# hermda02/dang

Measured on AMD Instinct MI355X. Metric: gibbs_iterations_per_sec, higher is better.
Workload: dtype f64

## Files before the change

### dang_amd/csrc/dangx_planeset.hip

```cpp
#ifndef DX_NO_VCOEF
#define DX_VCOEF 1
#endif
#include "dx_host.h"
#include "dx_kern_planeset.h"

static size_t planeset_lds(int ng, int nb, int nv, int lanes, int Sp) {
    const int rows = nv > Sp ? nv : Sp;
    return ((size_t)(TROWS * ng + 3) * nb + (size_t)rows * (nb / lanes) * BLOCK) * sizeof(double);
}

static void item_codes(const SweepList& sl, int code[4]) {
    for (int q = 0; q < 4; ++q) code[q] = (q < sl.n) ? sl.s[q].mode + 8 * sl.s[q].pair : 0;
}
static std::string planeset_name(int Sp, int nb, int ng, int lanes, int solve, const SweepList& sl, int bp) {
    int c[4];
    item_codes(sl, c);
    std::string s = "dxk::k_plane_set<" + std::to_string(Sp) + ", " + std::to_string(nb) + ", " + std::to_string(ng) + ", " + std::to_string(lanes) +
                    ", " + std::to_string(solve);
    for (int q = 0; q < 4; ++q) s += ", " + std::to_string(c[q]);
    return s + ", " + std::to_string(bp) + ">";
}

static int planeset_bp(dangx_ctx* ctx) {
    for (int j = 0; j < ctx->hm.nbands; ++j)
        if (ctx->hm.band[j].n != 0) return 1;
    return 0;
}

static bool planeset_builtin(int nb, int ng, int lanes, int solve, const SweepList& sl) {
    int c[4];
    item_codes(sl, c);
    if (nb == 20 && ng == 6 && lanes == 2) return solve && c[0] == CH_POW && c[1] == CH_MBB_BETA + 8 && c[2] == CH_LOGN_NUP && c[3] == 0;
    if (lanes == 1 && nb == 10 && ng == 4 && solve && sl.n == 0) return true;
    if (lanes == 1 && ((nb == 10 && ng == 4) || (solve && ((nb == 5 && ng == 3) || (nb == 3 && ng == 2)))))
        return c[0] == CH_POW && c[1] == CH_MBB_BETA + 8 && c[2] == 0 && c[3] == 0;
    return false;
}

template <int NB, int NG, int LP, int SOLVE, int C0, int C1, int C2>
static void launch_builtin(dangx_ctx* ctx, const GroupArgs& ga, const FusedArgs& fa, const SweepList& sl, int Sp, unsigned nblk, size_t ldsz,
                           unsigned long long* accp) {
    if (Sp == 2)
        hipLaunchKernelGGL((dxk::k_plane_set<2, NB, NG, LP, SOLVE, C0, C1, C2, 0>), dim3(nblk), dim3(BLOCK), ldsz, ctx->stream, ctx->dm, ga, fa, sl, ctx->counters, accp, ctx->partial);
    else
        hipLaunchKernelGGL((dxk::k_plane_set<1, NB, NG, LP, SOLVE, C0, C1, C2, 0>), dim3(nblk), dim3(BLOCK), ldsz, ctx->stream, ctx->dm, ga, fa, sl, ctx->counters, accp, ctx->partial);
}

static bool planeset_args(dangx_ctx* ctx, const GroupArgs& ga, const SweepList& sl, FusedArgs& fa) {
    fa.nv = 0; fa.gself = -1;
    unsigned planes = 0;
    for (int k = sl.s1; k <= sl.s2; ++k) planes |= 1u << (k - 1);
    for (int g = 0; g < MAXG; ++g) { fa.vslot[g] = -1; fa.vcomp[g] = 0; fa.vtype[g] = 0; }
    for (int g = 0; g < ga.ng; ++g) {
        const int l = ga.gc[g];
        const Comp& c = ctx->hm.comp[l];
        const unsigned cm = (unsigned)c.const_planes & planes;
        if (cm != 0 && cm != planes) return false;
        if (cm != planes) {
            if (c.type != DANGX_POWERLAW && c.type != DANGX_MBB && c.type != DANGX_FREEFREE && c.type != DANGX_LOGNORMAL) return false;
            if (sl.s2 > sl.s1 && (ctx->qu_equal[l] & ((1u << c.nind) - 1u)) != ((1u << c.nind) - 1u)) return false;
            fa.vcomp[fa.nv] = (signed char)g; fa.vtype[fa.nv] = (signed char)c.type;
            fa.vslot[g] = (signed char)fa.nv++;
        }
    }
    fa.cal = 0;
    if (sl.s1 == 1)
        for (int j = 0; j < ctx->hm.nbands; ++j)
            if (ctx->hm.gain[j] != 1.0 || ctx->hm.offset[j] != 0.0) fa.cal = 1;
    return true;
}

int dx_planeset_lanes(dangx_ctx* ctx, const GroupArgs& ga, const SweepList& sl, int solve) {
    static const bool enabled = [] { const char* e = getenv("DANGX_PLANESET"); return !(e && e[0] == '0'); }();
    static const bool small_too = [] { const char* e = getenv("DANGX_PLANESET"); return !(e && e[0] == 'p'); }();
    if (!enabled || sl.n < 0 || sl.n > 4 || (sl.n == 0 && !solve) || ga.ng < 1 || ga.ng > 6) return 0;
    static const int cap2 = [] { const char* e = getenv("DANGX_PS_CAP2"); return e ? atoi(e) : 13; }();
    const int nb = ctx->hm.nbands, Sp = sl.s2 - sl.s1 + 1, cap = (Sp == 2) ? cap2 : 16;
    for (int q = 0; q < sl.n; ++q) {
        const int m = sl.s[q].mode;
        if (m < CH_POW || m > CH_LOGN_W) return 0;
        if (sl.s[q].pair && !(m == CH_MBB_BETA || m == CH_LOGN_NUP)) return 0;
    }
    FusedArgs fa;
    if (!planeset_args(ctx, ga, sl, fa)) return 0;
    if (solve && fa.cal && ga.nuc > 0) return 0;
    const int bp = planeset_bp(ctx);
    if (bp) {
        for (int q = 0; q < sl.n; ++q)
            if (sl.s[q].mode > CH_MBB_T) return 0;
        if (!(small_too && nb <= cap && planeset_lds(ga.ng, nb, fa.nv, 1, Sp) <= 80u * 1024u)) return 0;
        return dx_rtc_get(ctx, "dx_kern_planeset.h", planeset_name(Sp, nb, ga.ng, 1, solve, sl, 1)) ? 1 : 0;
    }
    int lanes = 0;
    if (small_too && nb <= cap && planeset_lds(ga.ng, nb, fa.nv, 1, Sp) <= 80u * 1024u) lanes = 1;
    else if (nb > 12 && nb % 2 == 0 && nb / 2 <= cap && planeset_lds(ga.ng, nb, fa.nv, 2, Sp) <= 80u * 1024u) lanes = 2;
    if (!lanes) return 0;
    if (planeset_builtin(nb, ga.ng, lanes, solve, sl)) return lanes;
    return dx_rtc_get(ctx, "dx_kern_planeset.h", planeset_name(Sp, nb, ga.ng, lanes, solve, sl, 0)) ? lanes : 0;
}

bool dx_launch_planeset(dangx_ctx* ctx, const GroupArgs& ga, const SweepList& sl, int lanes, int solve, unsigned nblk, unsigned long long* accp) {
    FusedArgs fa;
    if (lanes < 1 || lanes > 2 || !planeset_args(ctx, ga, sl, fa)) return false;
    const int nb = ctx->hm.nbands, ng = ga.ng, Sp = sl.s2 - sl.s1 + 1;
    const size_t ldsz = planeset_lds(ng, nb, fa.nv, lanes, Sp);
    const int bp = planeset_bp(ctx);
    if (!bp && planeset_builtin(nb, ng, lanes, solve, sl)) {
        if (nb == 20) launch_builtin<20, 6, 2, 1, CH_POW, CH_MBB_BETA + 8, CH_LOGN_NUP>(ctx, ga, fa, sl, Sp, nblk, ldsz, accp);
        else if (nb == 10 && sl.n == 0) launch_builtin<10, 4, 1, 1, 0, 0, 0>(ctx, ga, fa, sl, Sp, nblk, ldsz, accp);
        else if (nb == 10 && !solve) launch_builtin<10, 4, 1, 0, CH_POW, CH_MBB_BETA + 8, 0>(ctx, ga, fa, sl, Sp, nblk, ldsz, accp);
        else if (nb == 10) launch_builtin<10, 4, 1, 1, CH_POW, CH_MBB_BETA + 8, 0>(ctx, ga, fa, sl, Sp, nblk, ldsz, accp);
        else if (nb == 5) launch_builtin<5, 3, 1, 1, CH_POW, CH_MBB_BETA + 8, 0>(ctx, ga, fa, sl, Sp, nblk, ldsz, accp);
        else launch_builtin<3, 2, 1, 1, CH_POW, CH_MBB_BETA + 8, 0>(ctx, ga, fa, sl, Sp, nblk, ldsz, accp);
        return true;
    }
    hipFunction_t fn = dx_rtc_get(ctx, "dx_kern_planeset.h", planeset_name(Sp, nb, ng, lanes, solve, sl, bp));
    if (!fn) return false;
    const Model* dm = ctx->dm;
    GroupArgs gg = ga;
    SweepList ss = sl;
    unsigned long long* bad = ctx->counters;
    double* part = ctx->partial;
    void* args[] = {&dm, &gg, &fa, &ss, &bad, &accp, &part};
    return dx_rtc_launch(ctx, fn, nblk, ldsz, args) == 0;
}
```

### dang_amd/csrc/dx_chain.h

```cpp
#pragma once
#include "dx_args.h"


template <bool V> struct BoolTag { static constexpr bool value = V; };

#ifdef DX_CHAIN_LIBEXP
#define CEXP(x) exp(x)
#define CEXPS(x) exp(x)
#define CEXP1(x) exp(x)
#else
#define CEXP(x) exp_nr(x)
#define CEXPS(x) exp_sat(x)
#define CEXP1(x) exp_nr_v(x)
#endif
#ifdef DX_CHAIN_IEEEDIV
#define CDIV(a, b) ((a) / (b))
#else
#define CDIV(a, b) ((a) * fast_rcp(b))
#endif

#ifndef DX_CHAIN_UNSCALED
#define DX_CHAIN_SCALED 1
#endif
#ifndef DX_CHAIN_PAIR_RNG
#define DX_CHAIN_PAIR_RNG 1
#endif

namespace {

__device__ __forceinline__ bool mh_accept(double diff, double u3) {
#if defined(DX_ACCEPT_FULL) || defined(DX_CHAIN_LIBEXP)
    return (diff >= 0.0) || (CEXP1(diff) > u3);
#else
    const float e = __builtin_amdgcn_exp2f((float)diff * 0x1.715476p+0f);
    const float uf = (float)u3;
    bool acc = (diff >= 0.0) || (e > uf * 0x1.001p+0f);
    const bool unsure = !(acc || e < uf * 0x1.ffep-1f);
    if (__builtin_amdgcn_ballot_w64(unsure) != 0ull) {
        if (unsure) acc = CEXP1(diff) > u3;
    }
    return acc;
#endif
}


template <int LP>
struct BandPick {
    int half;
    __device__ __forceinline__ double operator()(const double* arr, int j, int nbh) const {
        if (LP == 1) return arr[j];
        const double a = arr[j], b = arr[nbh + j];
        return half ? b : a;
    }
    __device__ __forceinline__ double nu_c(const Model& M, int j, int nbh) const {
        if (LP == 1) return M.band[j].nu_c;
        const double a = M.band[j].nu_c, b = M.band[nbh + j].nu_c;
        return half ? b : a;
    }
};

template <int MODE, int SP, int NB, int LP, bool KT = false, bool BP = false>
struct RegChain {
    static constexpr bool kBP = BP;
    double D[SP][NB], F[NB], ISr[SP][NB];
    double bpa, bpb;
    double K1[(LP > 1 && !KT) ? NB : 1], K2[(LP > 1 && !KT) ? NB : 1];
    const double *kt1, *kt2;
    double amp[SP];

    __device__ __forceinline__ double is(int kk, int j) const { return ISr[kk][j]; }
    __device__ __forceinline__ void set_is(int kk, int j, double v) { ISr[kk][j] = v; }
    __device__ __forceinline__ double k1(const Model& M, const Comp& c, int j) const {
        if (KT) return kt1[j];
        if (LP > 1) return K1[j];
        return (MODE == CH_MBB_T) ? M.band[j].nu_c : (MODE == CH_LOGN_NUP) ? c.lnu9[j] : c.lnr[j];
    }
    __device__ __forceinline__ double k2(const Comp& c, int j) const { return KT ? kt2[j] : (LP > 1) ? K2[j] : c.cst[j]; }
    __device__ __forceinline__ void set_kt(const double* tab, int nbands, int ng, int g, int jb) {
        kt1 = tab + ((MODE == CH_MBB_T) ? TROWS * ng : (MODE == CH_LOGN_NUP) ? TROWS * g + 2 : TROWS * g) * nbands + jb;
        kt2 = tab + (TROWS * g + 1) * nbands + jb;
    }
    __device__ __forceinline__ void set_k(const Model& M, const Comp& c, const BandPick<LP>& pick) {
        if (LP > 1 && !KT) {
#pragma unroll
            for (int j = 0; j < NB; ++j) {
                K1[j] = (MODE == CH_MBB_T) ? pick.nu_c(M, j, NB) : (MODE == CH_LOGN_NUP) ? pick(c.lnu9, j, NB) : pick(c.lnr, j, NB);
                K2[j] = (MODE == CH_LOGN_NUP || MODE == CH_LOGN_W) ? pick(c.cst, j, NB) : 0.0;
            }
        }
    }

    template <bool BATCH, int OP = 0>
    __device__ __forceinline__ double lnl(const Model& M, const Comp& c, double th, double other, double& acc0, double& acc1) {
        double s0 = 0.0, s1 = 0.0;
        if (MODE == CH_POW) s0 = th;
        else if (MODE == CH_MBB_BETA) s0 = th + 1.0;
        else if (MODE == CH_MBB_T) { s0 = mbb_z(th); s1 = CEXP(s0 * c.nu_ref) - 1.0; }
        else if (MODE == CH_LOGN_NUP) { s0 = log_pos(th); s1 = other; }
        else s1 = th;
        acc0 = 0.0; acc1 = 0.0;
#ifdef DX_CHAIN_IEEEDIV
        const double rs1 = 1.0 / s1;
#else
        const double rs1 = (MODE == CH_LOGN_NUP || MODE == CH_LOGN_W) ? fast_rcp(s1) : 0.0;
#endif
        constexpr int TT = BP ? 1 : (NB % 5 == 0) ? 5 : (NB % 4 == 0) ? 4 : (NB % 3 == 0) ? 3 : 1;
        static_assert(!BP || (LP == 1 && (MODE == CH_POW || MODE == CH_MBB_BETA || MODE == CH_MBB_T)), "bandpass chains: one lane, power law / mbb");
#pragma unroll
        for (int j0 = 0; j0 < NB; j0 += TT) {
            double s[TT];
            if (BP && M.band[j0].n != 0) {
                const Band& b = M.band[j0];
                const kptr nu = as_const(M.bp_nu0 + b.off);
                const kptr tau = as_const(M.bp_tau0 + b.off);
                const kptr lnr = as_const(c.bp_lnr + b.off);
                const int n = b.n;
                double sj = 0.0;
                if (MODE == CH_POW) {
#pragma unroll 4
                    for (int q = 0; q < n; ++q) sj = sj + tau[q] * CEXP(s0 * lnr[q]);
                } else if (MODE == CH_MBB_BETA) {
#pragma unroll 4
                    for (int q = 0; q < n; ++q) sj = sj + (tau[q] * bpb) * fast_rcp(CEXP(bpa * nu[q]) - 1.0) * CEXP(s0 * lnr[q]);
                } else {
#pragma unroll 4
                    for (int q = 0; q < n; ++q) sj = sj + (tau[q] * s1) * fast_rcp(CEXP(s0 * nu[q]) - 1.0) * CEXP(bpa * lnr[q]);
                }
                s[0] = sj;
            } else
            if (MODE == CH_MBB_T && TT > 1 && BATCH) {
                double den[TT], pre[TT];
#pragma unroll
                for (int t = 0; t < TT; ++t) den[t] = CEXP(s0 * k1(M, c, j0 + t)) - 1.0;
                pre[0] = den[0];
#pragma unroll
                for (int t = 1; t < TT; ++t) pre[t] = pre[t - 1] * den[t];
                double inv = s1 * fast_rcp(pre[TT - 1]);
#pragma unroll
                for (int t = TT - 1; t > 0; --t) {
                    s[t] = (inv * pre[t - 1]) * F[j0 + t];
                    inv *= den[t];
                }
                s[0] = inv * F[j0];
            } else
#pragma unroll
            for (int t = 0; t < TT; ++t) {
                const int j = j0 + t;
                if (MODE == CH_LOGN_NUP) {
                    const double l = (k1(M, c, j) - s0) * rs1;
                    s[t] = CEXPS(-0.5 * (l * l)) * k2(c, j);
                } else if (MODE == CH_LOGN_W) {
                    const double l = F[j] * rs1;
                    s[t] = CEXPS(-0.5 * (l * l)) * k2(c, j);
                } else {
                    const double e = CEXP(s0 * k1(M, c, j));
                    if (MODE == CH_POW) s[t] = e;
                    else if (MODE == CH_MBB_BETA) s[t] = F[j] * e;
                    else s[t] = CDIV(s1, e - 1.0) * F[j];
                }
            }
#pragma unroll
            for (int t = 0; t < TT; ++t) {
                const int j = j0 + t;
#ifdef DX_CHAIN_SCALED
                if (OP == 1) {
                    const double r0 = D[0][j];
                    D[0][j] = fma(is(0, j), s[t], r0);
                    acc0 = fma(r0, r0, acc0);
                    if (SP == 2) {
                        const double r1 = D[SP - 1][j];
                        D[SP - 1][j] = fma(is(SP - 1, j), s[t], r1);
                        acc1 = fma(r1, r1, acc1);
                    }
                } else if (OP == 2) {
                    D[0][j] = fma(-is(0, j), s[t], D[0][j]);
                    if (SP == 2) D[SP - 1][j] = fma(-is(SP - 1, j), s[t], D[SP - 1][j]);
                } else {
                const double r0 = fma(-is(0, j), s[t], D[0][j]);
                acc0 = fma(r0, r0, acc0);
                if (SP == 2) {
                    const double r1 = fma(-is(SP - 1, j), s[t], D[SP - 1][j]);
                    acc1 = fma(r1, r1, acc1);
                }
                }
#else
                const double r0 = (D[0][j] - amp[0] * s[t]) * is(0, j);
                acc0 = acc0 - 0.5 * (r0 * r0);
                if (SP == 2) {
                    const double r1 = (D[SP - 1][j] - amp[SP - 1] * s[t]) * is(SP - 1, j);
                    acc1 = acc1 - 0.5 * (r1 * r1);
                }
#endif
            }
        }
        if (OP == 2) return 0.0;
        if (LP > 1) {
            acc0 += __shfl_xor(acc0, 1, 64);
            if (SP == 2) acc1 += __shfl_xor(acc1, 1, 64);
        }
#ifdef DX_CHAIN_SCALED
        acc0 *= -0.5; acc1 *= -0.5;
#endif
        return acc0 + acc1;
    }
    __device__ __forceinline__ void scale() {
#ifdef DX_CHAIN_SCALED
#pragma unroll
        for (int kk = 0; kk < SP; ++kk)
#pragma unroll
            for (int j = 0; j < NB; ++j) { D[kk][j] *= ISr[kk][j]; ISr[kk][j] *= amp[kk]; }
#endif
    }
};

template <int NB, int LP>
__device__ __forceinline__ void subtract_other(const Model& M, const Comp& c2, int k, double amp2, double t0, double t1,
                                               double (&Dk)[NB], const BandPick<LP>& pick) {
    if ((c2.const_planes >> (k - 1)) & 1) {
#pragma unroll
        for (int j = 0; j < NB; ++j) Dk[j] -= amp2 * pick(c2.csed[k - 1], j, NB);
        return;
    }
    const Prep pr = sed_prep(c2, t0, t1);
    switch (c2.type) {
    case DANGX_POWERLAW:
#pragma unroll
        for (int j = 0; j < NB; ++j) Dk[j] -= amp2 * CEXP(pr.p0 * pick(c2.lnr, j, NB));
        break;
    case DANGX_MBB:
#pragma unroll
        for (int j = 0; j < NB; ++j) Dk[j] -= amp2 * (CDIV(pr.p2, CEXP(pr.p1 * pick.nu_c(M, j, NB)) - 1.0) * CEXP(pr.p0 * pick(c2.lnr, j, NB)));
        break;
    case DANGX_FREEFREE:
#pragma unroll
        for (int j = 0; j < NB; ++j) Dk[j] -= amp2 * (ff_gaunt(pick(c2.lnu9, j, NB), pr.p0) / pr.p1 * pick(c2.cst, j, NB));
        break;
    case DANGX_LOGNORMAL: {
        const double rp1 = fast_rcp(pr.p1);
#pragma unroll
        for (int j = 0; j < NB; ++j) {
            const double l2 = (pick(c2.lnu9, j, NB) - pr.p2) * rp1;
            Dk[j] -= amp2 * (CEXPS(-0.5 * (l2 * l2)) * pick(c2.cst, j, NB));
        }
        break;
    }
    default:
#pragma unroll
        for (int j = 0; j < NB; ++j) Dk[j] -= amp2 * pick(c2.cst, j, NB);
        break;
    }
}

template <int NB, int LP>
__device__ __forceinline__ void subtract_other_pair(const Model& M, const Comp& c2, double ampa, double ampb, double t0, double t1,
                                                    double (&Da)[NB], double (&Db)[NB], const BandPick<LP>& pick) {
    const Prep pr = sed_prep(c2, t0, t1);
    switch (c2.type) {
    case DANGX_POWERLAW:
#pragma unroll
        for (int j = 0; j < NB; ++j) { const double s = CEXP(pr.p0 * pick(c2.lnr, j, NB)); Da[j] -= ampa * s; Db[j] -= ampb * s; }
        break;
    case DANGX_MBB:
#pragma unroll
        for (int j = 0; j < NB; ++j) {
            const double s = CDIV(pr.p2, CEXP(pr.p1 * pick.nu_c(M, j, NB)) - 1.0) * CEXP(pr.p0 * pick(c2.lnr, j, NB));
            Da[j] -= ampa * s; Db[j] -= ampb * s;
        }
        break;
    case DANGX_FREEFREE:
#pragma unroll
        for (int j = 0; j < NB; ++j) {
            const double s = ff_gaunt(pick(c2.lnu9, j, NB), pr.p0) / pr.p1 * pick(c2.cst, j, NB);
            Da[j] -= ampa * s; Db[j] -= ampb * s;
        }
        break;
    case DANGX_LOGNORMAL: {
        const double rp1 = fast_rcp(pr.p1);
#pragma unroll
        for (int j = 0; j < NB; ++j) {
            const double l2 = (pick(c2.lnu9, j, NB) - pr.p2) * rp1;
            const double s = CEXPS(-0.5 * (l2 * l2)) * pick(c2.cst, j, NB);
            Da[j] -= ampa * s; Db[j] -= ampb * s;
        }
        break;
    }
    default:
#pragma unroll
        for (int j = 0; j < NB; ++j) { const double s = pick(c2.cst, j, NB); Da[j] -= ampa * s; Db[j] -= ampb * s; }
        break;
    }
}

template <int MODE, int SP, int NB, int LP, bool SCALE = true, bool ADD = false, bool SUB = false, class RC>
__device__ __forceinline__ unsigned long long chain_finish(const Model& M, const IndexArgs& a, const Comp& c, RC& R,
                                                           const BandPick<LP>& pick, double sample0, double sample1, int i, int half,
                                                           double chi[4], double* final_value = nullptr,
                                                           const double* acc_in = nullptr, double* acc_out = nullptr) {
    const int npix = M.npix;
    double* out = c.idx + ((long long)a.nind * M.nmaps) * npix + i;
    const bool first = (a.nind == 0);
    if (SCALE) R.scale();
    if (MODE == CH_MBB_BETA) {
        const double z = mbb_z(sample1);
        const double A = CEXP(z * c.nu_ref) - 1.0;
#pragma unroll
        for (int j = 0; j < NB; ++j) R.F[j] = CDIV(A, CEXP(z * pick.nu_c(M, j, NB)) - 1.0);
        if (RC::kBP) { R.bpa = z; R.bpb = A; }
    } else if (MODE == CH_MBB_T) {
#pragma unroll
        for (int j = 0; j < NB; ++j) R.F[j] = CEXP((sample0 + 1.0) * pick(c.lnr, j, NB));
        if (RC::kBP) R.bpa = sample0 + 1.0;
    } else if (MODE == CH_LOGN_W) {
        {
            const double lp = log_pos(sample0);
#pragma unroll
            for (int j = 0; j < NB; ++j) R.F[j] = pick(c.lnu9, j, NB) - lp;
        }
    }
    const double other = first ? sample1 : sample0;
    const unsigned long long gpix = (unsigned long long)(M.pix0 + i);
    const int q = a.nind;
    const bool gauss = c.prior_type[q] == DANGX_PRIOR_GAUSSIAN;
    const double pmean = c.gauss[q][0], pstd = c.gauss[q][1], lgden = c.lgden[q];
    const double inv2v = 1.0 / (2 * (pstd * pstd));
    auto prior = [&](double v) -> double {
        if (!gauss) return 0.0;
#ifdef DX_CHAIN_IEEEDIV
        const double arg = ((v - pmean) * (v - pmean)) / (2 * (pstd * pstd));
#else
        const double arg = ((v - pmean) * (v - pmean)) * inv2v;
#endif
        return (arg > 745.0) ? -INFINITY : -arg - lgden;
    };
    unsigned long long nacc = 0;
    double cur = first ? sample0 : sample1;
    double a0, a1, c0, c1;
    const double step = c.step[q], lo = c.uni[q][0], hi = c.uni[q][1];
    auto chain = [&](auto batch_tag) {
        constexpr bool B = decltype(batch_tag)::value;
        double lnl;
        if (acc_in) { a0 = acc_in[0]; a1 = acc_in[1]; lnl = a0 + a1; }
        else lnl = R.template lnl<B, ADD ? 1 : 0>(M, c, cur, other, a0, a1);
        chi[0] = -2.0 * a0; chi[1] = -2.0 * a1;
        double lnl_old = lnl + prior(cur);
        if (LP == 1 || DX_CHAIN_PAIR_RNG == 0) {
            for (int l = 1; l <= a.nsample; ++l) {
                double u1, u2, u3;
                uniform3(a.seed, a.stream, gpix, (uint32_t)l, u1, u2, u3);
                const double prop = cur + rand_normal(0.0, step, u1, u2);
                if (prop < lo || prop > hi) continue;
                lnl = R.template lnl<B>(M, c, prop, other, c0, c1);
                const double lnl_new = lnl + prior(prop);
                const double diff = lnl_new - lnl_old;
                const bool acc = (a.ml_mode == DANGX_ML_OPTIMIZE) ? (diff > 0.0) : mh_accept(diff, u3);
                if (acc) { cur = prop; lnl_old = lnl_new; a0 = c0; a1 = c1; ++nacc; }
            }
        } else {
            auto mh_step = [&](double g, double u3) {
                const double prop = cur + g;
                if (prop < lo || prop > hi) return;
                lnl = R.template lnl<B>(M, c, prop, other, c0, c1);
                const double lnl_new = lnl + prior(prop);
                const double diff = lnl_new - lnl_old;
                const bool acc = (a.ml_mode == DANGX_ML_OPTIMIZE) ? (diff > 0.0) : mh_accept(diff, u3);
                if (acc) { cur = prop; lnl_old = lnl_new; a0 = c0; a1 = c1; ++nacc; }
            };
            for (int l = 1; l <= a.nsample; l += 2) {
                double u1, u2, u3;
                uniform3(a.seed, a.stream, gpix, (uint32_t)(l + half), u1, u2, u3);
                const double g = rand_normal(0.0, step, u1, u2);
                const double go = __shfl_xor(g, 1, 64), uo = __shfl_xor(u3, 1, 64);
                mh_step(half == 0 ? g : go, half == 0 ? u3 : uo);
                if (l + 1 <= a.nsample) mh_step(half == 0 ? go : g, half == 0 ? uo : u3);
            }
        }
        if (SUB) { double u0_, u1_; (void)R.template lnl<B, 2>(M, c, cur, other, u0_, u1_); }
    };
#ifdef DX_CHAIN_NO_BATCH_RCP
    chain(BoolTag<false>{});
#else
    if (MODE == CH_MBB_T && !RC::kBP) {
        const double tmin = fmin(lo, cur);
#ifdef DX_BATCH_ALWAYS
        chain(BoolTag<true>{});
#elif defined(DX_BATCH_LANEWISE)
        if (tmin > 0.0 && mbb_z(tmin) * M.mbb_batch_z < 1.0) chain(BoolTag<true>{});
        else chain(BoolTag<false>{});
#else
        const bool unsafe = !(tmin > 0.0 && mbb_z(tmin) * M.mbb_batch_z < 1.0);
        if (__builtin_amdgcn_ballot_w64(unsafe) == 0ull) chain(BoolTag<true>{});
        else chain(BoolTag<false>{});
#endif
    } else {
        chain(BoolTag<false>{});
    }
#endif
    if (final_value) *final_value = cur;
    if (acc_out) { acc_out[0] = a0; acc_out[1] = a1; }
    if (half != 0) {
        chi[0] = chi[1] = 0.0;
        return 0ull;
    }
#pragma unroll
    for (int kk = 0; kk < SP; ++kk) out[(long long)(a.s1 + kk - 1) * npix] = cur;
    chi[2] = -2.0 * a0; chi[3] = -2.0 * a1;
    return nacc;
}

template <int MODE, int SP, int NB, int LP>
__device__ __forceinline__ void index_chain_stage(const Model& M, const IndexArgs& a, const Comp& c, RegChain<MODE, SP, NB, LP>& R,
                                                  const BandPick<LP>& pick, int i, double& sample0, double& sample1) {
    const int npix = M.npix;
    const int jb = pick.half * NB;
    R.set_k(M, c, pick);
    load_theta(M, c, i, a.s1, sample0, sample1);
    const long long bstride = (long long)M.nmaps * npix;
#pragma unroll
    for (int kk = 0; kk < SP; ++kk) {
        const int k = a.s1 + kk;
        R.amp[kk] = c.amp[(long long)(k - 1) * npix + i];
        const double* sigp = M.sig + (long long)(k - 1) * npix + i;
        const double* rmsp = M.rms + (long long)(k - 1) * npix + i;
        double rv[NB];
#pragma unroll
        for (int j = 0; j < NB; ++j) {
            R.D[kk][j] = sigp[(jb + j) * bstride];
            rv[j] = rmsp[(jb + j) * bstride];
        }
#pragma unroll
        for (int j = 0; j < NB; ++j) {
            if (k == 1) R.D[kk][j] = (R.D[kk][j] - pick(M.offset, j, NB)) / pick(M.gain, j, NB);
            R.set_is(kk, j, CDIV(1.0, rv[j]));
        }
    }
    {
        unsigned om = a.others;
        double na[SP], nt0[SP], nt1[SP];
        auto fetch = [&](int l) {
            const Comp& c2 = M.comp[l];
#pragma unroll
            for (int kk = 0; kk < SP; ++kk) {
                na[kk] = c2.amp[(long long)(a.s1 + kk - 1) * npix + i];
                nt0[kk] = nt1[kk] = 0.0;
                if (!((c2.const_planes >> (a.s1 + kk - 1)) & 1)) load_theta(M, c2, i, a.s1 + kk, nt0[kk], nt1[kk]);
            }
        };
        int l = om ? __builtin_ctz(om) : -1;
        if (l >= 0) fetch(l);
        while (l >= 0) {
            const Comp& c2 = M.comp[l];
            double ca[SP], ct0[SP], ct1[SP];
#pragma unroll
            for (int kk = 0; kk < SP; ++kk) { ca[kk] = na[kk]; ct0[kk] = nt0[kk]; ct1[kk] = nt1[kk]; }
            om &= om - 1;
            const int ln = om ? __builtin_ctz(om) : -1;
            if (ln >= 0) fetch(ln);
            const unsigned cp = (c2.const_planes >> (a.s1 - 1)) & 3u;
            if (SP == 2 && cp == 0 && ct0[0] == ct0[SP - 1] && ct1[0] == ct1[SP - 1]) {
                subtract_other_pair<NB, LP>(M, c2, ca[0], ca[SP - 1], ct0[0], ct1[0], R.D[0], R.D[SP - 1], pick);
            } else {
#pragma unroll
                for (int kk = 0; kk < SP; ++kk) subtract_other<NB, LP>(M, c2, a.s1 + kk, ca[kk], ct0[kk], ct1[kk], R.D[kk], pick);
            }
            l = ln;
        }
    }
}

template <int MODE, int SP, int NB, int LP>
__device__ __forceinline__ unsigned long long index_chain_reg(const Model& M, const IndexArgs& a, int i, int half, double chi[4]) {
    const int npix = M.npix;
    const Comp& c = M.comp[a.comp];
    double* out = c.idx + ((long long)a.nind * M.nmaps) * npix + i;
    if (is_masked(M.mask[i])) {
        if (half == 0) {
#pragma unroll
            for (int kk = 0; kk < SP; ++kk) out[(long long)(a.s1 + kk - 1) * npix] = 0.0;
        }
        return 0ull;
    }
    const BandPick<LP> pick = {half};
    RegChain<MODE, SP, NB, LP> R;
    double sample0, sample1;
    index_chain_stage<MODE, SP, NB, LP>(M, a, c, R, pick, i, sample0, sample1);
    return chain_finish<MODE, SP, NB, LP>(M, a, c, R, pick, sample0, sample1, i, half, chi);
}

template <int MODEA, int MODEB, int SP, int NB, int LP>
__device__ __forceinline__ void index_chain_pair(const Model& M, const IndexArgs& a, const IndexArgs& b, int i, int half, double chi[4],
                                                 unsigned long long& nacc_a, unsigned long long& nacc_b) {
    const int npix = M.npix;
    const Comp& c = M.comp[a.comp];
    nacc_a = nacc_b = 0ull;
    if (is_masked(M.mask[i])) {
        if (half == 0) {
#pragma unroll
            for (int kk = 0; kk < SP; ++kk) {
                c.idx[((long long)a.nind * M.nmaps + (a.s1 + kk - 1)) * npix + i] = 0.0;
                c.idx[((long long)b.nind * M.nmaps + (a.s1 + kk - 1)) * npix + i] = 0.0;
            }
        }
        return;
    }
    const BandPick<LP> pick = {half};
    RegChain<MODEA, SP, NB, LP> RA;
    double sample0, sample1;
    index_chain_stage<MODEA, SP, NB, LP>(M, a, c, RA, pick, i, sample0, sample1);
    double chia[4] = {0.0, 0.0, 0.0, 0.0}, chib[4] = {0.0, 0.0, 0.0, 0.0}, va;
    nacc_a = chain_finish<MODEA, SP, NB, LP>(M, a, c, RA, pick, sample0, sample1, i, half, chia, &va);
    RegChain<MODEB, SP, NB, LP> RB;
    RB.set_k(M, c, pick);
#pragma unroll
    for (int kk = 0; kk < SP; ++kk) {
        RB.amp[kk] = RA.amp[kk];
#pragma unroll
        for (int j = 0; j < NB; ++j) { RB.D[kk][j] = RA.D[kk][j]; RB.ISr[kk][j] = RA.ISr[kk][j]; }
    }
    if (a.nind == 0) sample0 = va; else sample1 = va;
    nacc_b = chain_finish<MODEB, SP, NB, LP, false>(M, b, c, RB, pick, sample0, sample1, i, half, chib);
    chi[0] = chia[0]; chi[1] = chia[1]; chi[2] = chib[2]; chi[3] = chib[3];
}

}
```

Before: 90.76.

## Certify Metropolis-Hastings decisions with a cheap float-exp likelihood and rigorous error bound

Adds a low-precision likelihood evaluation that uses float exp2/rcp, plus a per-chain error bound on it. When the bound shows the accept/reject decision is certain, the full f64 likelihood is skipped. Only wavefronts with an undecided lane fall back to the exact evaluation, and the exact chi-square sums are recomputed at the end if the last accepted state came from the cheap path. The OP==2 subtract path now also accumulates residuals so those sums come for free. This trades extra bound arithmetic and wavefront divergence for fewer f64 exp evaluations, and correctness depends on the error bounds being sound.

```diff
diff --git a/dang_amd/csrc/dangx_planeset.hip b/dang_amd/csrc/dangx_planeset.hip
--- a/dang_amd/csrc/dangx_planeset.hip
+++ b/dang_amd/csrc/dangx_planeset.hip
@@ -124,3 +124,11 @@
     void* args[] = {&dm, &gg, &fa, &ss, &bad, &accp, &part};
     return dx_rtc_launch(ctx, fn, nblk, ldsz, args) == 0;
 }
+
+#ifdef DX_LNL_DIAG
+extern "C" int dangx_lnl_diag(unsigned long long* out) {
+    if (hipMemcpyFromSymbol(out, HIP_SYMBOL(g_lnl_diag), 2 * sizeof(unsigned long long)) != hipSuccess) return 1;
+    const unsigned long long z[2] = {0ull, 0ull};
+    return hipMemcpyToSymbol(HIP_SYMBOL(g_lnl_diag), z, sizeof(z)) == hipSuccess ? 0 : 1;
+}
+#endif
diff --git a/dang_amd/csrc/dx_chain.h b/dang_amd/csrc/dx_chain.h
--- a/dang_amd/csrc/dx_chain.h
+++ b/dang_amd/csrc/dx_chain.h
@@ -43,6 +43,21 @@
 #endif
 }
 
+__device__ __forceinline__ bool mh_certain(double dlo, double dhi, double u3, bool& acc) {
+    const float uf = (float)u3;
+    const float elo = __builtin_amdgcn_exp2f((float)dlo * 0x1.715476p+0f);
+    const float ehi = __builtin_amdgcn_exp2f((float)dhi * 0x1.715476p+0f);
+    acc = (dlo >= 0.0) || (elo > uf * 0x1.001p+0f);
+    return acc || ((dhi < 0.0) && (ehi < uf * 0x1.ffep-1f));
+}
+
+
+#ifdef DX_LNL_DIAG
+__device__ unsigned long long g_lnl_diag[2];
+__device__ __forceinline__ void lnl_diag_count(int k) {
+    if (__lane_id() == __builtin_ctzll(__builtin_amdgcn_ballot_w64(true))) atomicAdd(&g_lnl_diag[k], 1ull);
+}
+#endif
 
 template <int LP>
 struct BandPick {
@@ -173,8 +188,14 @@
                         acc1 = fma(r1, r1, acc1);
                     }
                 } else if (OP == 2) {
-                    D[0][j] = fma(-is(0, j), s[t], D[0][j]);
-                    if (SP == 2) D[SP - 1][j] = fma(-is(SP - 1, j), s[t], D[SP - 1][j]);
+                    const double r0 = fma(-is(0, j), s[t], D[0][j]);
+                    D[0][j] = r0;
+                    acc0 = fma(r0, r0, acc0);
+                    if (SP == 2) {
+                        const double r1 = fma(-is(SP - 1, j), s[t], D[SP - 1][j]);
+                        D[SP - 1][j] = r1;
+                        acc1 = fma(r1, r1, acc1);
+                    }
                 } else {
                 const double r0 = fma(-is(0, j), s[t], D[0][j]);
                 acc0 = fma(r0, r0, acc0);
@@ -193,7 +214,6 @@
 #endif
             }
         }
-        if (OP == 2) return 0.0;
         if (LP > 1) {
             acc0 += __shfl_xor(acc0, 1, 64);
             if (SP == 2) acc1 += __shfl_xor(acc1, 1, 64);
@@ -202,6 +222,59 @@
         acc0 *= -0.5; acc1 *= -0.5;
 #endif
         return acc0 + acc1;
+    }
+
+    __device__ __forceinline__ double lnl_cheap(const Model& M, const Comp& c, double th) {
+        double s0 = 0.0, s1 = 0.0;
+        if (MODE == CH_POW) s0 = th;
+        else if (MODE == CH_MBB_BETA) s0 = th + 1.0;
+        else { s0 = mbb_z(th); s1 = CEXP(s0 * c.nu_ref) - 1.0; }
+        const double s0l = s0 * 0x1.71547652b82fep+0;
+        double acc0 = 0.0, acc1 = 0.0;
+#pragma unroll
+        for (int j = 0; j < NB; ++j) {
+            const float e = __builtin_amdgcn_exp2f((float)(s0l * k1(M, c, j)));
+            double s;
+            if (MODE == CH_POW) s = (double)e;
+            else if (MODE == CH_MBB_BETA) s = F[j] * (double)e;
+            else s = (s1 * F[j]) * (double)__builtin_amdgcn_rcpf(e - 1.0f);
+            const double r0 = fma(-is(0, j), s, D[0][j]);
+            acc0 = fma(r0, r0, acc0);
+            if (SP == 2) {
+                const double r1 = fma(-is(SP - 1, j), s, D[SP - 1][j]);
+                acc1 = fma(r1, r1, acc1);
+            }
+        }
+        double a = acc0 + acc1;
+        if (LP > 1) a += __shfl_xor(a, 1, 64);
+        return a;
+    }
+
+    __device__ __forceinline__ bool cheap_bound(const Model& M, const Comp& c, double lo, double hi, double a_start,
+                                                double& wA, double& wG) {
+        double G = 0.0, emax = 0.0, kmax = 0.0;
+        double smax, zmin = 0.0;
+        if (MODE == CH_POW) smax = fmax(fabs(lo), fabs(hi));
+        else if (MODE == CH_MBB_BETA) smax = fmax(fabs(lo + 1.0), fabs(hi + 1.0));
+        else { smax = mbb_z(lo); zmin = mbb_z(hi); }
+#pragma unroll
+        for (int j = 0; j < NB; ++j) {
+            const double k = fabs(k1(M, c, j));
+            kmax = fmax(kmax, k);
+            double e;
+            if (MODE == CH_MBB_T) e = (1.0 + smax * k) * 0x1p-24 + (2.0 + (double)__builtin_amdgcn_rcpf((float)(zmin * k))) * 0x1p-22;
+            else e = (smax * k) * 0x1p-24 + 0x1p-22;
+            e = e * (1.0 + 0x1p-8) + 0x1p-46;
+            emax = fmax(emax, e);
+#pragma unroll
+            for (int kk = 0; kk < SP; ++kk) { const double t = e * D[kk][j]; G = fma(t, t, G); }
+        }
+        if (LP > 1) { G += __shfl_xor(G, 1, 64); emax = fmax(emax, __shfl_xor(emax, 1, 64)); kmax = fmax(kmax, __shfl_xor(kmax, 1, 64)); }
+        const double lam = fmax(sqrt(G * fast_rcp(fmax(a_start, 0x1p-900))), 0x1p-400);
+        wA = 0.5 * ((2.0 * emax * (1.0 + emax) + lam) * (1.0 + 0x1p-40) + 0x1p-40);
+        wG = 0.5 * ((G * fast_rcp(lam) + 2.0 * G) * (1.0 + 0x1p-40) + 0x1p-1000);
+        const bool range = smax * kmax * 0x1.71547652b82fep+0 <= 125.0;
+        return (MODE == CH_MBB_T) ? (range && lo > 0.0 && zmin > 0.0) : range;
     }
     __device__ __forceinline__ void scale() {
 #ifdef DX_CHAIN_SCALED
@@ -336,6 +409,12 @@
     double cur = first ? sample0 : sample1;
     double a0, a1, c0, c1;
     const double step = c.step[q], lo = c.uni[q][0], hi = c.uni[q][1];
+    const bool ml_opt = (a.ml_mode == DANGX_ML_OPTIMIZE);
+#if defined(DX_LNL_EXACT) || !defined(DX_CHAIN_SCALED)
+    constexpr bool kCert = false;
+#else
+    constexpr bool kCert = !RC::kBP && (MODE == CH_POW || MODE == CH_MBB_BETA || MODE == CH_MBB_T);
+#endif
     auto chain = [&](auto batch_tag) {
         constexpr bool B = decltype(batch_tag)::value;
         double lnl;
@@ -343,38 +422,87 @@
         else lnl = R.template lnl<B, ADD ? 1 : 0>(M, c, cur, other, a0, a1);
         chi[0] = -2.0 * a0; chi[1] = -2.0 * a1;
         double lnl_old = lnl + prior(cur);
+        bool cert = false, old_exact = true, sums_exact = true;
+        double wA = 0.0, wG = 0.0, wold = 0.0;
+        if (kCert) {
+            const bool ok = R.cheap_bound(M, c, lo, hi, -2.0 * lnl, wA, wG) && !ml_opt;
+            cert = __builtin_amdgcn_ballot_w64(!ok) == 0ull;
+        }
+        auto mh_step = [&](double prop, double u3) {
+            if (prop < lo || prop > hi) return;
+            if constexpr (!kCert) {
+                lnl = R.template lnl<B>(M, c, prop, other, c0, c1);
+                const double lnl_new = lnl + prior(prop);
+                const double diff = lnl_new - lnl_old;
+                const bool acc = ml_opt ? (diff > 0.0) : mh_accept(diff, u3);
+                if (acc) { cur = prop; lnl_old = lnl_new; a0 = c0; a1 = c1; ++nacc; }
+            } else {
+                const double pp = prior(prop);
+                bool acc = false, und = true;
+                double lc = 0.0, wc = 0.0;
+                if (cert) {
+                    const double A = R.lnl_cheap(M, c, prop);
+                    lc = -0.5 * A;
+                    wc = fma(wA, A, wG);
+                    const double dc = (lc + pp) - lnl_old;
+                    const double W = (wc + wold) * (1.0 + 0x1p-40) + 0x1p-49 * ((fabs(lc) + fabs(pp)) + fabs(lnl_old));
+                    und = !mh_certain(dc - W, dc + W, u3, acc);
+#ifdef DX_LNL_DIAG
+                    lnl_diag_count(0);
+                    if (__builtin_amdgcn_ballot_w64(und) != 0ull) lnl_diag_count(1);
+#endif
+                }
+                if (__builtin_amdgcn_ballot_w64(und) != 0ull) {
+                    if (und) {
+                        bool again = !old_exact;
+#pragma unroll 1
+                        for (;;) {
+                            const double l = R.template lnl<B>(M, c, again ? cur : prop, other, c0, c1);
+                            if (!again) { lnl = l; break; }
+                            lnl_old = l + prior(cur);
+                            again = false;
+                        }
+                        const double lnl_new = lnl + pp;
+                        const double diff = lnl_new - lnl_old;
+                        acc = ml_opt ? (diff > 0.0) : mh_accept(diff, u3);
+                        if (acc) { lnl_old = lnl_new; a0 = c0; a1 = c1; }
+                        old_exact = true;
+                        wold = 0.0;
+                    }
+                }
+                if (acc) {
+                    cur = prop;
+                    ++nacc;
+                    sums_exact = und;
+                    if (!und) { lnl_old = lc + pp; wold = wc; old_exact = false; }
+                }
+            }
+        };
         if (LP == 1 || DX_CHAIN_PAIR_RNG == 0) {
             for (int l = 1; l <= a.nsample; ++l) {
                 double u1, u2, u3;
                 uniform3(a.seed, a.stream, gpix, (uint32_t)l, u1, u2, u3);
-                const double prop = cur + rand_normal(0.0, step, u1, u2);
-                if (prop < lo || prop > hi) continue;
-                lnl = R.template lnl<B>(M, c, prop, other, c0, c1);
-                const double lnl_new = lnl + prior(prop);
-                const double diff = lnl_new - lnl_old;
-                const bool acc = (a.ml_mode == DANGX_ML_OPTIMIZE) ? (diff > 0.0) : mh_accept(diff, u3);
-                if (acc) { cur = prop; lnl_old = lnl_new; a0 = c0; a1 = c1; ++nacc; }
+                mh_step(cur + rand_normal(0.0, step, u1, u2), u3);
             }
         } else {
-            auto mh_step = [&](double g, double u3) {
-                const double prop = cur + g;
-                if (prop < lo || prop > hi) return;
-                lnl = R.template lnl<B>(M, c, prop, other, c0, c1);
-                const double lnl_new = lnl + prior(prop);
-                const double diff = lnl_new - lnl_old;
-                const bool acc = (a.ml_mode == DANGX_ML_OPTIMIZE) ? (diff > 0.0) : mh_accept(diff, u3);
-                if (acc) { cur = prop; lnl_old = lnl_new; a0 = c0; a1 = c1; ++nacc; }
-            };
             for (int l = 1; l <= a.nsample; l += 2) {
                 double u1, u2, u3;
                 uniform3(a.seed, a.stream, gpix, (uint32_t)(l + half), u1, u2, u3);
                 const double g = rand_normal(0.0, step, u1, u2);
                 const double go = __shfl_xor(g, 1, 64), uo = __shfl_xor(u3, 1, 64);
-                mh_step(half == 0 ? g : go, half == 0 ? u3 : uo);
-                if (l + 1 <= a.nsample) mh_step(half == 0 ? go : g, half == 0 ? uo : u3);
-            }
-        }
-        if (SUB) { double u0_, u1_; (void)R.template lnl<B, 2>(M, c, cur, other, u0_, u1_); }
+                mh_step(cur + (half == 0 ? g : go), half == 0 ? u3 : uo);
+                if (l + 1 <= a.nsample) mh_step(cur + (half == 0 ? go : g), half == 0 ? uo : u3);
+            }
+        }
+        if (SUB) {
+            double s0_, s1_;
+            (void)R.template lnl<B, 2>(M, c, cur, other, s0_, s1_);
+            if (!sums_exact) { a0 = s0_; a1 = s1_; }
+        } else if (kCert) {
+            if (__builtin_amdgcn_ballot_w64(!sums_exact) != 0ull) {
+                if (!sums_exact) (void)R.template lnl<B>(M, c, cur, other, a0, a1);
+            }
+        }
     };
 #ifdef DX_CHAIN_NO_BATCH_RCP
     chain(BoolTag<false>{});
```

Result: faster. 98.42, median of 6 (+8.4%).
